# snsinfu/2022a-genome-dynamics

Hardware: AMD Instinct MI355X
Metric: bead-steps/sec on 100kb whole-genome model, 1 GPU and 8-GPU replica farm (higher is better)
Workload: dtype f32

## Files before the change

2022a-genome-dynamics_amd/__init__.py:

```python
from __future__ import annotations

import ctypes as C
import os
from dataclasses import dataclass

import numpy as np

_HERE = os.path.dirname(os.path.abspath(__file__))
LIBGDYN_PATH = os.path.join(_HERE, "csrc", "libgdyn.so")

GD_BOX_OPEN, GD_BOX_PERIODIC = 0, 1
POT_HARMONIC, POT_SPRING, POT_SEMISPRING, POT_SOFTCORE = 0, 1, 2, 3
NOISE_PHILOX, NOISE_ZERO, NOISE_HOST, NOISE_MT19937 = 0, 1, 2, 3
RUN_UPDATE_SCALES, RUN_WALL_DYNAMICS, RUN_DEFER_CALLBACK, RUN_COMPENSATED, RUN_UNCOMPENSATED = 1, 2, 4, 8, 16
ALL_REPLICAS = 0xffffffff
ABI_VERSION = 5
TERM_PAIR, TERM_BOND, TERM_BEND, TERM_POINT, TERM_WALL, TERM_DYNAMIC, TERM_ALL = 1, 2, 4, 8, 16, 32, 63

_STATUS = {1: "GD_EINVAL", 2: "GD_ENODEVICE", 3: "GD_EHIP", 4: "GD_ENOMEM", 5: "GD_ESTATE", 6: "GD_EUNSUPPORTED"}


class GdynError(RuntimeError):
    def __init__(self, code, msg):
        super().__init__(f"{_STATUS.get(code, code)}: {msg}")
# ... 302 lines not shown
        return out

    def forces(self, terms=TERM_ALL):
        out = np.empty((self.R, self.N, 3))
        self.lib.check(self.lib.dll.gd_compute_forces(self._h, terms, _dptr(out)))
        return out

    def search_pairs(self, dcut, replica=0):
        n = C.c_uint64(0)
        self.lib.check(self.lib.dll.gd_search_pairs(self._h, replica, dcut, None, 0, C.byref(n)))
        out = np.empty((n.value, 2), dtype=np.uint32)
        if n.value:
            self.lib.check(self.lib.dll.gd_search_pairs(self._h, replica, dcut, _uptr(out), n.value, C.byref(n)))
        return out

    def contacts_update(self, distance):
        self.lib.check(self.lib.dll.gd_contacts_update(self._h, distance))

    def contacts(self, replica=0):
        n = C.c_uint64(0)
        self.lib.check(self.lib.dll.gd_contacts_fetch(self._h, replica, None, 0, C.byref(n)))
        out = np.empty((n.value, 3), dtype=np.uint32)
        if n.value:
            self.lib.check(self.lib.dll.gd_contacts_fetch(self._h, replica, _uptr(out), n.value, C.byref(n)))
        return out

    def contacts_clear(self, replica=ALL_REPLICAS):
        self.lib.check(self.lib.dll.gd_contacts_clear(self._h, replica))

    def set_tuning(self, skin=0.0, rebuild_interval=0, adapt_interval=1, list_width=0, kernel_path=0, near_fraction=0.0, auto_skin=0):
        t = Tuning(skin, rebuild_interval, adapt_interval, list_width, kernel_path, near_fraction, auto_skin)
        self.lib.check(self.lib.dll.gd_set_tuning(self._h, C.byref(t)))

    def timing(self):
        t = Timing()
        self.lib.check(self.lib.dll.gd_get_timing(self._h, C.byref(t)))
        return t

    def debug_bench(self, what, n=20):
        f = getattr(self.lib.dll, "gd_debug_bench", None)
        if f is None:
            raise GdynError(6, "gd_debug_bench: not in this library (developer builds only: make -C csrc dev; load('libgdyn_dev.so'))")
        f.argtypes = [C.c_void_p, C.c_int, C.c_int, C.POINTER(C.c_double)]
        ms = C.c_double(0)
        self.lib.check(f(self._h, what, n, C.byref(ms)))
        return ms.value

    def stream(self):
        p = C.c_void_p()
        self.lib.check(self.lib.dll.gd_get_stream(self._h, C.byref(p)))
        return p.value
```

2022a-genome-dynamics_amd/csrc/gdyn_capi.hip:

```cpp
#include <algorithm>
#include <cmath>
#include <cstdarg>
#include <cstdio>
#include <cstdlib>
#include <cstring>
#include <new>
#include <string>
#include <vector>

#include "../../include/gdyn.h"
#include "../../include/gdyn_replica.h"
#include "../../include/gdyn_ensemble.h"
#include <hip/hip_fp16.h>

#include "gdyn_types.h"
#include "gdyn_once.hpp"
#include "gdyn_policy.hpp"
#include "gdyn_list.hpp"
#include "gdyn_live.hpp"
#include "gdyn_replica_pairs.hpp"
#include "gdyn_ensemble.hpp"
#include "gdyn_glue.hpp"
#include "gdyn_glue_types.h"
#include "../../include/gdyn_glue.h"
#ifdef GD_DEV
#include "gdyn_dev.h"
#endif


static thread_local char g_err[1024];
static int fail(int code, const char *fmt, ...)
{
    va_list ap;
    va_start(ap, fmt);
    vsnprintf(g_err, sizeof g_err, fmt, ap);
    va_end(ap);
    return code;
}
#define HIPCHK(call)                                                                                    \
    do {                                                                                                \
        hipError_t e_ = (call);                                                                         \
        if (e_ != hipSuccess) return fail(GD_EHIP, "%s failed: %s (%s:%d)", #call, hipGetErrorString(e_), __FILE__, __LINE__); \
    } while (0)
#define GDCHK(call)              \
    do {                         \
// ... 86 lines not shown

    DevBuf<float2> ab_o; uint32_t ab_stride = 0;
    DevBuf<float> mob_o; DevBuf<float4> bendE_o; DevBuf<unsigned char> psmask_o, bdeg_o;
    DevBuf<unsigned> badj_o; DevBuf<int4> chain_o; DevBuf<BondType> btab;
    DevBuf<float4> pos[2], xb, fout, snap;
    DevBuf<unsigned> orig[2], slot_of, rank, members, cell_cnt, cell_start, nbr, meta, badj, flags;
    DevBuf<float> bbox_enc, bbox_w;
    DevBuf<unsigned short> nbr16; DevBuf<TileDesc> tiles;
    DevBuf<float4> rec_x0; DevBuf<uint2> rec_mo; DevBuf<unsigned char> len_prev;
    DevBuf<uint2> wtab, rqueue; DevBuf<unsigned short> need_prev; DevBuf<unsigned> pool;
    DevBuf<float> bbox;
    DevBuf<float2> ab; DevBuf<float> mobs; DevBuf<float4> bendE; DevBuf<int4> chain;
    float mob_uniform = -1.f;
    DevBuf<GridP> grid; DevBuf<DevCtx> ctx[2]; DevBuf<float4> react_part[2]; DevBuf<double> epart;
    DevBuf<unsigned long long> lcount_d; DevBuf<float> noise;
    DevBuf<unsigned long long> seeds_d;
    DevBuf<unsigned> dmax;
    double last_dt = 0, last_kT = -1;
    int last_flags = 0;
    double pend_dt = 0; int pend_flags = 0;
    double near_frac = 0.65;
    DevBuf<uint2> sp_out; DevBuf<unsigned long long> sp_count; std::vector<uint2> sp_host;
    bool sp_valid = false; uint32_t sp_r = 0; double sp_dcut = 0; uint64_t sp_serial = 0;
    DevBuf<unsigned long long> ct_words; DevBuf<unsigned> ct_distinct; size_t ct_cap = 0;
    DevBuf<uint2> ct_pairs; DevBuf<unsigned long long> ct_count; std::vector<unsigned> ct_distinct_h;
    DevBuf<unsigned long long> ct_ck[2]; DevBuf<unsigned> ct_cv[2], ct_n; DevBuf<char> ct_tmp;
    uint64_t state_serial = 1;
    int ocur = 0;
    DevBuf<float4> lo, snap_lo;
    bool lo_valid = false;
    bool comp_last = false;
    double mob_max = 1.0;
    std::vector<hipEvent_t> events;
    ~gd_system()
    {
        for (auto e : events) (void)hipEventDestroy(e);
        if (rp_copied) (void)hipEventDestroy(rp_copied);
        if (stream) (void)hipStreamDestroy(stream);
    }
};

static int valid_pq(int p, int q) { return (p == 2 || p == 4 || p == 6 || p == 8 || p == 12) && q >= 1 && q <= 4; }

extern "C" int gd_abi_version(void) { return GD_ABI_VERSION; }

extern "C" int gd_create_abi(int abi_version, const gd_desc *d, gd_system **out)
{
    if (abi_version != GD_ABI_VERSION)
        return fail(GD_EINVAL, "gd_create: the caller was built against gdyn.h ABI version %d, this library implements %d", abi_version, GD_ABI_VERSION);
    if (!d || !out) return fail(GD_EINVAL, "gd_create: NULL argument");
    if (d->n_beads == 0 || d->n_replicas == 0) return fail(GD_EINVAL, "gd_create: n_beads and n_replicas must be > 0");
    if (d->n_beads > GD_ADJ_MASK) return fail(GD_EINVAL, "gd_create: n_beads exceeds %u", GD_ADJ_MASK);
    if (d->box_kind != GD_BOX_OPEN && d->box_kind != GD_BOX_PERIODIC) return fail(GD_EINVAL, "gd_create: bad box_kind");
    if (d->box_kind == GD_BOX_PERIODIC)
        for (int k = 0; k < 3; k++) if (!(d->box[k] > 0)) return fail(GD_EINVAL, "gd_create: periodic box needs positive periods");
    int ndev = 0;
    if (hipGetDeviceCount(&ndev) != hipSuccess || ndev == 0)
        return fail(GD_ENODEVICE, "gd_create: no HIP device visible (libgdyn has no CPU fallback)");
    if (d->device < 0 || d->device >= ndev) return fail(GD_ENODEVICE, "gd_create: device %d not in [0,%d)", d->device, ndev);
    HIPCHK(hipSetDevice(d->device));
    {
        static gd::DeviceOnce<> once;
        const int rc = once.run(d->device, [](int) { return (int)gd_kernels_init_device(); });
        if (rc != (int)hipSuccess)
            return fail(GD_EHIP, "gd_create: kernel set-up on device %d failed: %s", d->device, rc < 0 ? "device ordinal beyond the guard's table" : hipGetErrorString((hipError_t)rc));
    }
    gd_system *s = new (std::nothrow) gd_system();
    if (!s) return fail(GD_ENOMEM, "gd_create: out of host memory");
    s->N = d->n_beads; s->R = d->n_replicas; s->device = d->device; s->box_kind = d->box_kind;
// ... 457 lines not shown
        if (s->has_scaling) { c.bead_scale = s->bs_init; c.bond_scale = s->bo_init; }
        if (semi) memcpy(c.semi, semi + 3 * r, sizeof c.semi);
    }
    s->ctx_dirty = true; s->list.drop();
    return GD_OK;
}

extern "C" int gd_set_context(gd_system *s, uint32_t r, int64_t step, double bead_scale, double bond_scale, const double semi[3])
{
    if (!s) return fail(GD_EINVAL, "gd_set_context: NULL system");
    if (r >= s->R) return fail(GD_EINVAL, "gd_set_context: replica out of range");
    if (!(bead_scale > 0) || !(bond_scale > 0)) return fail(GD_EINVAL, "gd_set_context: scales must be positive");
    DevCtx &c = s->hctx[r];
    c.step = step; c.bead_scale = bead_scale; c.bond_scale = bond_scale; c.pending = 0;
    if (semi) memcpy(c.semi, semi, sizeof c.semi);
    s->ctx_dirty = true; s->list.drop();
    return GD_OK;
}

extern "C" int gd_set_tuning(gd_system *s, const gd_tuning *t)
{
    if (!s || !t) return fail(GD_EINVAL, "gd_set_tuning: NULL argument");
    if (t->kernel_path > 2) return fail(GD_EINVAL, "gd_set_tuning: kernel_path must be 0..2");
    if (t->near_fraction < 0 || t->near_fraction > 1) return fail(GD_EINVAL, "gd_set_tuning: near_fraction must be in [0,1]");
    HIPCHK(hipSetDevice(s->device));
    if (s->pol.set_tuning(t->skin, t->rebuild_interval, t->adapt_interval, t->list_width, t->auto_skin != 0 || dev_env("GDYN_AUTO_SKIN")))
        (void)s->nbr.resize(0);
    if (t->near_fraction > 0) s->near_frac = t->near_fraction;
    s->kernel_path = t->kernel_path;
    s->list.drop();
    return GD_OK;
}
extern "C" int gd_get_timing(gd_system *s, gd_timing *o) { if (!s || !o) return fail(GD_EINVAL, "gd_get_timing: NULL"); *o = s->timing; return GD_OK; }
extern "C" int gd_get_stream(gd_system *s, void **st) { if (!s || !st) return fail(GD_EINVAL, "gd_get_stream: NULL"); *st = (void *)s->stream; return GD_OK; }


static float pair_cutoff(const gd_system *s)
{
    double m = 0;
    if (s->has_pair) {
        if (s->pair.eps_a != 0 && s->pair.sigma_a > m) m = s->pair.sigma_a;
        if (s->pair.eps_b != 0 && s->pair.sigma_b > m) m = s->pair.sigma_b;
    }
    return (float)m;
}

static int finalize_topology(gd_system *s)
{
    if (!s->topo_dirty) return GD_OK;
    HIPCHK(hipSetDevice(s->device));
    const uint32_t N = s->N;
    std::vector<gd_bond_params> types = s->btypes;
    std::vector<int> terms = s->bterm;
    std::vector<Bond> all = s->bonds;
    for (int d = 0; d < 4; d++) if (s->dyn[d].used) {
        if (types.size() >= GD_MAX_BOND_TYPES) return fail(GD_EINVAL, "too many bond parameter sets");
        types.push_back(s->dyn[d].p); terms.push_back(GD_TERM_DYNAMIC);
        const int t = (int)types.size() - 1;
        for (size_t k = 0; k + 1 < s->dyn[d].pairs.size(); k += 2) all.push_back({s->dyn[d].pairs[k], s->dyn[d].pairs[k + 1], t});
    }
    const bool hetero = !s->ens.homogeneous();
    s->bonds_premixed = false;
    if (!hetero) {
        std::vector<gd_bond_params> t2; std::vector<int> term2; std::vector<Bond> all2 = all;
        bool fits = true, any_mixed = false;
        for (auto &b : all2) {
// ... 80 lines not shown
    s->n_bond_types = (uint32_t)bt.size();
    const size_t RNp = (size_t)s->R * s->Np;
    const uint32_t WBp = std::max((WB + 3u) & ~3u, 4u);
    if (WBp != s->WB || !s->badj.p) { HIPCHK(s->badj.resize((size_t)WBp * RNp)); }
    if (has_bend && !s->chain.p) { HIPCHK(s->chain.resize(RNp)); HIPCHK(s->bendE.resize(RNp)); }
    s->WB = WBp; s->has_bend = has_bend; s->has_bonds = !all.empty();
    s->mob_uniform = (float)s->mob[0];
    for (uint32_t i = 1; i < N; i++) if ((float)s->mob[i] != s->mob_uniform) { s->mob_uniform = -1.f; break; }
    s->mob_max = 0;
    for (uint32_t i = 0; i < N; i++) s->mob_max = std::max(s->mob_max, s->mob[i]);
    s->topo_dirty = false; s->list.topology_changed();
    return GD_OK;
}


static double scale_at(const gd_system *s, double init, double tau, double time) { (void)s; return 1.0 - (1.0 - init) * std::exp(-time / tau); }

static double cut_scale(const gd_system *s, const gd_run_desc *run, uint32_t ahead)
{
    if (!s->pair.scale_by_bead_scale) return 1.0;
    double m = 0;
    for (auto &c : s->hctx) {
        m = std::max(m, c.bead_scale);
        if (run && (run->flags & GD_RUN_UPDATE_SCALES) && s->has_scaling)
            m = std::max(m, scale_at(s, s->bs_init, s->bs_tau, (double)(c.step + ahead + 1) * run->timestep));
    }
    return m;
}

static void fill_common(gd_system *s, StepParams &p)
{
    memset(&p, 0, sizeof p);
    p.N = s->N; p.Np = s->Np; p.R = s->R; p.nblk = s->nblk; p.stride = (size_t)s->R * s->Np;
    set_box(s, p);
    p.pos_in = s->pos[s->pcur].p; p.pos_out = s->pos[s->pcur ^ 1].p; p.xb = s->xb.p; p.orig = s->orig[s->ocur].p;
    p.ab = s->ab.p; p.mob = s->mobs.p; p.bendE = s->bendE.p; p.mob_uniform = s->mob_uniform; p.WB = s->WB;
    p.nbr = s->nbr.p; p.nbr16 = s->nbr16.p; p.wtab = s->wtab.p; p.tiles = s->tiles.p; p.tiled = s->list.tiled ? 1 : 0; p.packed_ab = s->packed_ab ? 1 : 0;
    p.cpb = s->cpb; p.tile_cap = s->list.tiled ? s->list.tile_cap : s->pol.tile_cap;
    p.pk = (s->has_pair && s->pair.p_a == 2 && s->pair.q_a == 3 && s->pair.p_b == 8 && s->pair.q_b == 3) ? (s->pair.mix ? 1 : 2) : 0;
    p.meta = s->meta.p; p.rec_x0 = s->rec_x0.p; p.rec_mo = s->rec_mo.p; p.W = s->list.W; p.badj = s->badj.p; p.chain = s->chain.p;
    p.ctx_in = s->ctx[s->ccur].p; p.ctx_out = s->ctx[s->ccur ^ 1].p; p.flags = s->flags.p;
    p.react_in = s->react_part[s->ccur].p; p.react_out = s->react_part[s->ccur ^ 1].p;
    if (s->has_pair) {
        const gd_pair_softcore &q = s->pair;
        p.pair = PairP{(float)q.eps_a, (float)q.sigma_a, (float)q.eps_b, (float)q.sigma_b, q.p_a, q.q_a, q.p_b, q.q_b,
                       q.mix, q.scale_by_bead_scale, pair_cutoff(s) > 0 ? 1 : 0, pair_cutoff(s)};
    }
    if (s->has_wall) {
        const gd_wall &w = s->wall;
        p.wall.eps_a = (float)w.eps_a; p.wall.sigma_a = (float)w.sigma_a; p.wall.eps_b = (float)w.eps_b; p.wall.sigma_b = (float)w.sigma_b;
        p.wall.p_a = w.p_a; p.wall.q_a = w.q_a; p.wall.p_b = w.p_b; p.wall.q_b = w.q_b;
        p.wall.wall_a = (float)w.wall_a_factor; p.wall.wall_b = (float)w.wall_b_factor; p.wall.scaled = w.scale_by_bead_scale;
        p.wall.enabled = 1; p.wall.packing_spring = (float)w.packing_spring;
        p.wall.fast2383 = (w.p_a == 2 && w.q_a == 3 && w.p_b == 8 && w.q_b == 3) ? 1 : 0;
        for (int k = 0; k < 3; k++) p.wall.spring[k] = w.semiaxes_spring[k];
        p.wall.mobility = w.mobility;
    }
    if (s->has_inner) {
        const gd_inner_sphere &w = s->inner;
        p.wall.inner_enabled = 1; p.wall.in_radius = (float)w.radius;
        p.wall.in_eps_a = (float)w.eps_a; p.wall.in_sigma_a = (float)w.sigma_a; p.wall.in_eps_b = (float)w.eps_b; p.wall.in_sigma_b = (float)w.sigma_b;
        p.wall.in_p_a = w.p_a; p.wall.in_q_a = w.q_a; p.wall.in_p_b = w.p_b; p.wall.in_q_b = w.q_b;
        p.wall.in_wall_a = (float)w.wall_a_factor; p.wall.in_wall_b = (float)w.wall_b_factor; p.wall.in_spring = (float)w.spring;
    }
    p.scaling = ScaleP{s->has_scaling ? 1 : 0, 0, s->bs_init, s->bs_tau, s->bo_init, s->bo_tau, 0.0, 0.0};
    p.btab = s->btab.p; p.nbt = (int)s->n_bond_types; p.has_softcore_bonds = s->has_softcore_bonds ? 1 : 0;
// ... 177 lines not shown
    fill_common(s, p);
    p.dt_d = s->pend_dt; p.dt = (float)s->pend_dt; p.run_flags = s->pend_flags;
    bool common = s->has_scaling && (s->pend_flags & GD_RUN_UPDATE_SCALES);
    for (uint32_t r = 1; r < s->R && common; r++) common = s->hctx[r].step == s->hctx[0].step && s->hctx[r].pending == s->hctx[0].pending;
    if (common) {
        const double time = (double)(s->hctx[0].step + 1) * s->pend_dt;
        p.scaling.from_host = 1;
        p.scaling.bead_next = scale_at(s, s->bs_init, s->bs_tau, time);
        p.scaling.bond_next = scale_at(s, s->bo_init, s->bo_tau, time);
    }
    gd_launch_finalize(p, 0, s->stream);
    s->ccur ^= 1;
    GDCHK(download_ctx(s));
    s->state_serial++;
    return GD_OK;
}

static bool want_compensated(const gd_system *s, const gd_run_desc *run)
{
    if (run->flags & GD_RUN_UNCOMPENSATED) return false;
    if (run->flags & GD_RUN_COMPENSATED) return true;
    double X = 0;
    if (s->has_wall) for (auto &c : s->hctx) for (int k = 0; k < 3; k++) X = std::max(X, c.semi[k]);
    if (s->box_kind == GD_BOX_PERIODIC) for (int k = 0; k < 3; k++) X = std::max(X, s->box[k]);
    if (!(X > 0)) X = 16.0;
    const double ulp = std::ldexp(1.0, std::ilogb(X) - 23), sigma = std::sqrt(2.0 * s->mob_max * run->temperature * run->timestep);
    return sigma < 64.0 * ulp;
}

extern "C" int gd_apply_callback(gd_system *s)
{
    if (!s) return fail(GD_EINVAL, "gd_apply_callback: NULL system");
    return apply_pending(s);
}

static int enqueue_chunk(gd_system *s, const gd_run_desc *run, int64_t done, bool comp, bool host_noise, Chunk &c)
{
    const size_t RN = (size_t)s->R * s->N;
    const bool with_list = pair_cutoff(s) > 0;
    const int64_t chunk = c.steps = s->pol.chunk_steps(run->steps - done);
    gd_launch_gather_positions(s->pos[s->pcur].p, s->slot_of.p, s->snap.p, s->N, s->Np, s->R, 0, s->stream);
    if (comp) HIPCHK(hipMemcpyAsync(s->snap_lo.p, s->lo.p, RN * sizeof(float4), hipMemcpyDeviceToDevice, s->stream));
    c.snap_ctx = s->hctx; c.snap_w_packed = s->list.w_packed;
    GDCHK(clear_flags(s));
    StepParams p;
    bool common_step = s->has_scaling && (run->flags & GD_RUN_UPDATE_SCALES);
    const long long step0 = s->hctx[0].step;
    for (uint32_t r = 1; r < s->R && common_step; r++) common_step = s->hctx[r].step == step0;
    auto host_scales = [&](StepParams &q, int64_t launch) {
        if (!common_step) return;
        const double time = (double)(step0 + launch) * run->timestep;
        q.scaling.from_host = 1;
        q.scaling.bead_next = scale_at(s, s->bs_init, s->bs_tau, time);
        q.scaling.bond_next = scale_at(s, s->bo_init, s->bo_tau, time);
    };
    size_t nev = 0;
    HIPCHK(hipEventRecord(get_event(s, nev++), s->stream));
    int64_t k = 0;
    c.on_search_list = s->list.valid && s->list.search_list;
    while (k < chunk) {
        if (!s->list.valid || s->list.steps_since_build >= s->pol.K) {
            s->pol.take_pending_skin(pair_cutoff(s));
            hipEvent_t e1 = get_event(s, nev++);
            GDCHK(enqueue_build(s, list_radius(s, run, (uint32_t)(k + s->pol.K)), with_list));
            s->list.enter_use(false);
            HIPCHK(hipEventRecord(e1, s->stream));
            c.spans.push_back({nev - 1, 1});
        }
        const int64_t n = std::min<int64_t>((int64_t)s->pol.K - s->list.steps_since_build, chunk - k);
        hipEvent_t e1 = get_event(s, nev++);
        for (int64_t q = 0; q < n; q++) {
            fill_common(s, p);
            p.dt_d = run->timestep; p.dt = (float)run->timestep; p.kT = (float)run->temperature; p.seed = run->seed;
            p.seeds = run->replica_seeds ? s->seeds_d.p : nullptr;
            p.noise_mode = run->noise_mode; p.run_flags = run->flags; p.comp = comp ? 1 : 0;
            p.host_noise = host_noise ? s->noise.p + (size_t)(done + k + q) * RN * 3 : nullptr;
            host_scales(p, k + q);
            p.record_disp = (s->list.steps_since_build + (uint32_t)q + 1u == s->pol.K);
            c.full_interval |= p.record_disp != 0;
            gd_launch_step(p, GD_MODE_STEP, s->stream);
            if (s->sw_n) launch_softwell(s, p, 0);
            if (s->rp.any()) launch_replica_pairs(s, p, 0);
            s->pcur ^= 1; s->ccur ^= 1;
        }
        HIPCHK(hipEventRecord(e1, s->stream));
        c.spans.push_back({nev - 1, 0});
        s->timing.step_launches += (uint64_t)n;
        s->list.stepped((uint32_t)n);
        k += n;
    }
    const bool defer = (run->flags & GD_RUN_DEFER_CALLBACK) && done + chunk == run->steps;
    if (!defer) {
        fill_common(s, p);
        p.dt_d = run->timestep; p.dt = (float)run->timestep; p.run_flags = run->flags;
        host_scales(p, chunk);
        gd_launch_finalize(p, 0, s->stream);
        s->ccur ^= 1;
    } else {
        s->pend_dt = run->timestep; s->pend_flags = run->flags;
        if (s->has_wall) {
            fill_common(s, p);
            p.ctx_out = s->ctx[s->ccur].p;
            gd_launch_finalize(p, 1, s->stream);
        }
    }
    c.ev_end = nev;
    HIPCHK(hipEventRecord(get_event(s, nev++), s->stream));
    return GD_OK;
}

static int rollback_chunk(gd_system *s, const Chunk &c, bool over, bool comp, int retries)
{
    const size_t RN = (size_t)s->R * s->N;
    s->rollbacks++;
    HIPCHK(hipMemcpy2DAsync(s->pos[s->pcur].p, (size_t)s->Np * sizeof(float4), s->snap.p, (size_t)s->N * sizeof(float4),
                            (size_t)s->N * sizeof(float4), s->R, hipMemcpyDeviceToDevice, s->stream));
    gd_launch_identity(s->orig[s->ocur].p, s->slot_of.p, s->N, s->Np, s->R, s->stream);
// ... 24 lines not shown
        HIPCHK(hipEventElapsedTime(&ms, s->events[sp.first - 1], s->events[sp.first]));
        (sp.second ? build_ms : step_ms) += ms;
    }
    HIPCHK(hipEventElapsedTime(&ms, s->events[0], s->events[c.ev_end]));
    s->timing.total_ms += ms; s->timing.step_kernel_ms += step_ms; s->timing.rebuild_ms += build_ms;
    s->hctx = c.ctx;
    unsigned long long L = 0; for (uint32_t r = 0; r < s->R; r++) L += s->lcount[r];
    s->timing.list_entries_visited += L * (uint64_t)c.steps;
    const gd::Accepted a{ms, c.steps, c.rep.maxd2, cut_scale(s, nullptr, 0), c.full_interval, c.on_search_list};
    if (s->pol.on_accepted(list_state(s), a, [&](uint32_t ahead) { return cut_scale(s, run, ahead); })) s->list.drop();
    return GD_OK;
}

extern "C" int gd_run(gd_system *s, const gd_run_desc *run)
{
    if (!s || !run) return fail(GD_EINVAL, "gd_run: NULL argument");
    if (run->spacestep != 0) return fail(GD_EUNSUPPORTED, "gd_run: spacestep != 0 (adaptive timestep) is not supported");
    if (run->steps < 0 || !(run->timestep > 0) || run->temperature < 0) return fail(GD_EINVAL, "gd_run: bad steps/timestep/temperature");
    if (run->noise_mode < 0 || run->noise_mode > GD_NOISE_HOST)
        return fail(run->noise_mode == 3 ? GD_EUNSUPPORTED : GD_EINVAL, "gd_run: noise_mode %d not available on the device", run->noise_mode);
    if (run->noise_mode == GD_NOISE_HOST && !run->host_noise) return fail(GD_EINVAL, "gd_run: host noise requested without array");
    if ((run->flags & GD_RUN_WALL_DYNAMICS) && !s->has_wall) return fail(GD_ESTATE, "gd_run: wall dynamics requested without a wall");
    if ((run->flags & GD_RUN_UPDATE_SCALES) && !s->has_scaling) return fail(GD_ESTATE, "gd_run: scale updates requested without gd_set_scaling");
    GDCHK(prepare(s));
    GDCHK(apply_pending(s));
    s->state_serial++;
    if (run->timestep != s->last_dt || run->temperature != s->last_kT) { s->pol.a2_ema = 0; s->last_dt = run->timestep; s->last_kT = run->temperature; }
    if (s->pol.adapt && s->pol.K > 4 && ((run->flags ^ s->last_flags) & (GD_RUN_WALL_DYNAMICS | GD_RUN_UPDATE_SCALES)) != 0 && s->rebuilds > 0)
        s->pol.K -= s->pol.K / 5;
    s->last_flags = run->flags;
    const bool with_list = pair_cutoff(s) > 0;
    const size_t RN = (size_t)s->R * s->N;
    memset(&s->timing, 0, sizeof s->timing);

    const bool host_noise = run->noise_mode == GD_NOISE_HOST && run->temperature > 0;
    if (host_noise) {
        const size_t n = (size_t)run->steps * RN * 3;
        std::vector<float> h(n);
        for (size_t i = 0; i < n; i++) h[i] = (float)run->host_noise[i];
        HIPCHK(s->noise.resize(n, false));
        HIPCHK(hipMemcpy(s->noise.p, h.data(), n * sizeof(float), hipMemcpyHostToDevice));
    }

    const bool comp = run->steps > 0 && want_compensated(s, run);
    if (comp) {
        if (!s->lo_valid) { HIPCHK(hipMemsetAsync(s->lo.p, 0, RN * sizeof(float4), s->stream)); s->lo_valid = true; }
        HIPCHK(s->snap_lo.resize(RN, false));
    }
    if (run->steps > 0) s->comp_last = comp;
    if (run->steps > 0 && !comp) s->lo_valid = false;

    if (run->replica_seeds) {
        static_assert(sizeof(unsigned long long) == sizeof(uint64_t), "seed width");
        HIPCHK(s->seeds_d.resize(s->R, false));
        HIPCHK(hipMemcpy(s->seeds_d.p, run->replica_seeds, s->R * sizeof(uint64_t), hipMemcpyHostToDevice));
    }

    int64_t done = 0;
    int retries = 0;
    s->pol.retries_over(false);
    float last_dmax2 = 0;
    while (done < run->steps) {
        Chunk c;
        GDCHK(enqueue_chunk(s, run, done, comp, host_noise, c));
        GDCHK(read_chunk(s, c));
        const bool over = s->pol.on_report(list_state(s), c.rep);
// ... 496 lines not shown
```

2022a-genome-dynamics_amd/csrc/gdyn_kernels.hip:

```cpp
#include <hip/hip_fp16.h>

#include <algorithm>

#include "gdyn_types.h"

#include "gdyn_stamps.h"

#if GD_ABL == 40 || GD_ABL == 41 || GD_ABL == 43
#define GD_REPLAY 1
constexpr bool RP_MEM = (GD_ABL == 40), RP_ALU = (GD_ABL == 41 || GD_ABL == 43);
#define GD_CONSUME4(v) asm volatile("" :: "v"((v).x), "v"((v).y), "v"((v).z), "v"((v).w))
#define GD_LAUNDER4(v) asm volatile("" : "+v"((v).x), "+v"((v).y), "+v"((v).z), "+v"((v).w))
#endif

#define TERM_PAIR 1u
#define TERM_BOND 2u
#define TERM_BEND 4u
#define TERM_POINT 8u
#define TERM_WALL 16u
#define TERM_DYNAMIC 32u
#define RUN_UPDATE_SCALES 1
#define RUN_WALL_DYNAMICS 2
#define NOISE_PHILOX 0
#define NOISE_ZERO 1
// ... 408 lines not shown
    const float mu_dt = mu * p.dt;
    const float sg = s_ctx.sg_uniform >= 0.f ? s_ctx.sg_uniform : sqrtf(2.0f * p.kT * mu_dt);
    const float ex = mu_dt * F.x + sg * z.x, ey = mu_dt * F.y + sg * z.y, ez = mu_dt * F.z + sg * z.z;
    float nx = xi.x + ex, ny = xi.y + ey, nz = xi.z + ez;
    if (p.comp) {
        float4 *lp = p.lo + ((size_t)r * p.N + bead.oid);
        const float4 l = *lp;
        const float tx = l.x + ex, ty = l.y + ey, tz = l.z + ez;
        nx = xi.x + tx; ny = xi.y + ty; nz = xi.z + tz;
        const float bx = nx - xi.x, by = ny - xi.y, bz = nz - xi.z;
        *lp = make_float4((xi.x - (nx - bx)) + (tx - bx), (xi.y - (ny - by)) + (ty - by), (xi.z - (nz - bz)) + (tz - bz), 0.f);
    }
    if (TILED) *(float4 *)((char *)(p.pos_out + bead.rbase + (size_t)blk * GD_BLOCK) + bead.local * 16u) = make_float4(nx, ny, nz, bead.xi4.w);
    else p.pos_out[bead.g] = make_float4(nx, ny, nz, bead.xi4.w);
    float dnew2 = 0.f;
    if (TILED) { const float e2 = ex * ex + ey * ey + ez * ez; dnew2 = (disp2 + e2 + 2.0f * __builtin_amdgcn_sqrtf(disp2 * e2)) * 1.000002f; }
    return dnew2;
}

template <int MODE, bool PERIODIC, bool TILED, int PK, bool S16, bool SPLIT = false>
#ifndef GD_STEP_WAVES
#define GD_STEP_WAVES 8
#endif
__global__ __launch_bounds__(GD_BLOCK, (TILED && MODE == GD_MODE_STEP) ? (S16 ? GD_STEP_WAVES : 4) : 1) void k_step(const StepParams p)
{
    extern __shared__ __attribute__((aligned(16))) float4 s_tile[];
    __shared__ BondType s_bt[GD_MAX_BOND_TYPES];
    __shared__ CtxF s_ctx;
    __shared__ float s_red[GD_BLOCK / 64][4];
    __shared__ double s_e[GD_BLOCK / 64];

    unsigned r, blk;
    if (!block_map(blockIdx.x, p.nblk, p.cpb, r, blk)) return;
    if (TILED && SPLIT) {
        const unsigned held = p.tiles[(size_t)r * p.nblk + blk].total;
        if (held <= p.tile_lo || held > p.tile_hi) return;
    }
    const unsigned tid = threadIdx.x, lane = tid & 63, wid = tid >> 6;
    const size_t rbase = (size_t)r * p.Np;
    const float4 *__restrict__ rpos = p.pos_in + rbase;

    GD_STAMP_BEGIN();
    const long long ctx_step0 = p.ctx_in[r].step;
    const int ctx_pending0 = p.ctx_in[r].pending;
    const float dmax0 = (MODE == GD_MODE_STEP && TILED) ? __uint_as_float(p.dmax[r * GD_DMAX_STRIDE]) : 0.f;
    const size_t gw6 = (rbase + blk * GD_BLOCK) / 64 + (size_t)(unsigned)__builtin_amdgcn_readfirstlane((int)wid);
    const uint2 wrow = TILED ? p.wtab[gw6] : make_uint2(0u, 0u);
    const unsigned NCL = TILED ? wrow.y : p.W / 4, NCB = p.WB / 4;
    uint2 mo = make_uint2(0u, 0u);
    float4 rec = make_float4(0.f, 0.f, 0.f, 0.f);
    uint4 adj0 = make_uint4(0, 0, 0, 0), qa = adj0, qb = adj0;
    unsigned own_base = 0, tile_ok = 0;
    if (TILED) {
        const size_t tbase = rbase + (size_t)blk * GD_BLOCK;
        mo = *(const uint2 *)((const char *)(p.rec_mo + tbase) + tid * 8u);
        const TileDesc *td = p.tiles + (size_t)r * p.nblk + blk;
        unsigned tlen[GD_TILE_RANGES], tst[GD_TILE_RANGES];
#pragma unroll
        for (int k = 0; k < GD_TILE_RANGES; k++) { tlen[k] = td->len[k]; tst[k] = td->start[k]; }
        own_base = td->own_base; tile_ok = td->nranges;
        asm volatile("" : "+v"(mo.x), "+v"(mo.y));
        GD_STAMP(9);
        {
            constexpr bool W0_FREE = MODE == GD_MODE_STEP;
            const unsigned wq = (unsigned)__builtin_amdgcn_readfirstlane((int)((W0_FREE ? (wid == 0 ? 0x100000u : wid - 1u) : wid) * 64u));
            constexpr unsigned DMA_STRIDE = W0_FREE ? GD_BLOCK - 64u : GD_BLOCK;
// ... 400 lines not shown
            const float4 v = p.react_in[(size_t)r * p.nblk + b];
            rx += v.x; ry += v.y; rz += v.z;
        }
        c.react[0] = wave_sum_d(rx); c.react[1] = wave_sum_d(ry); c.react[2] = wave_sum_d(rz);
    } else if (c.pending) {
        apply_callback(c, p, r, lane);
    }
    if (lane == 0) p.ctx_out[r] = c;
}

typedef void (*StepKernel)(StepParams);
template <int MODE, bool SPLIT, bool PER, bool TIL, bool S16>
static StepKernel step_kernel_pk(int pk)
{
    return pk == 1 ? k_step<MODE, PER, TIL, 1, S16, SPLIT> : pk == 2 ? k_step<MODE, PER, TIL, 2, S16, SPLIT> : k_step<MODE, PER, TIL, 0, S16, SPLIT>;
}
template <int MODE, bool SPLIT>
static StepKernel tiled_step_kernel(bool periodic, int pk, bool s16)
{
    static_assert(!SPLIT || MODE == GD_MODE_STEP, "only stepping is split by tile class");
    if (periodic) return s16 ? step_kernel_pk<MODE, SPLIT, true, true, true>(pk) : step_kernel_pk<MODE, SPLIT, true, true, false>(pk);
    return s16 ? step_kernel_pk<MODE, SPLIT, false, true, true>(pk) : step_kernel_pk<MODE, SPLIT, false, true, false>(pk);
}
template <int MODE>
static StepKernel step_kernel(bool periodic, bool tiled, int pk, bool s16)
{
    if (tiled) return tiled_step_kernel<MODE, false>(periodic, pk, s16);
    return periodic ? step_kernel_pk<MODE, false, true, false, false>(pk) : step_kernel_pk<MODE, false, false, false, false>(pk);
}

template <int MODE>
static void launch_step_mode(const StepParams &p, hipStream_t st)
{
    const dim3 grid(p.cpb ? GD_XCDS * p.cpb * p.R : p.R * p.nblk), block(GD_BLOCK);
    const size_t lds = p.tiled ? (size_t)p.tile_cap * sizeof(float4) : 0;
    const bool s16 = p.tiled && gd_tile_s16(p.tile_cap);
    const unsigned split_at = !p.tiled ? 0u : (s16 && p.tile_cap > 3312u) ? 3312u : (!s16 && p.tile_cap > 5072u) ? 5072u : (!s16 && p.tile_cap > 3312u) ? 3312u : 0u;
    if (MODE == GD_MODE_STEP && split_at) {
        const StepKernel k = tiled_step_kernel<GD_MODE_STEP, true>(p.periodic, p.pk, s16);
        StepParams q = p;
        for (int half = 0; half < 2; half++) {
            q.tile_cap = half ? p.tile_cap : split_at; q.tile_lo = half ? split_at : 0u; q.tile_hi = half ? 0xffffffffu : split_at;
            hipLaunchKernelGGL(k, grid, block, (size_t)q.tile_cap * sizeof(float4), st, q);
        }
        return;
    }
    const StepKernel k = step_kernel<MODE>(p.periodic, p.tiled, p.pk, s16);
    hipLaunchKernelGGL(k, grid, block, lds, st, p);
}

void gd_launch_step(const StepParams &p, int mode, hipStream_t st)
{
    if (mode == GD_MODE_STEP) launch_step_mode<GD_MODE_STEP>(p, st);
    else if (mode == GD_MODE_FORCE) launch_step_mode<GD_MODE_FORCE>(p, st);
    else launch_step_mode<GD_MODE_ENERGY>(p, st);
}

void gd_launch_finalize(const StepParams &p, int mode, hipStream_t st)
{
    hipLaunchKernelGGL(k_ctx, dim3(p.R), dim3(64), 0, st, p, mode);
}


template <int CTRL, int ROW_MASK>
__device__ __forceinline__ float dppi(float v, float ident)
{
    return __int_as_float(__builtin_amdgcn_update_dpp(__float_as_int(ident), __float_as_int(v), CTRL, ROW_MASK, 0xf, false));
// ... 1357 lines not shown
```

2022a-genome-dynamics_amd/csrc/gdyn_policy.hpp:

```cpp
#pragma once
#include <algorithm>
#include <cmath>
#include <cstdint>
#include <cstdio>
#include <cstring>
#include <vector>

#include "gdyn_types.h"

namespace gd {

struct BuildReport {
    unsigned bits = 0;
    bool over = false, class_over = false, tile_over = false, violated = false;
    unsigned need_w = 0, need_t = 0, ncell = 0;
    float maxd2 = 0;
};

inline BuildReport summarize(const unsigned *flags, uint32_t R)
{
    BuildReport b;
    for (const unsigned *f = flags; f < flags + (size_t)R * GD_NFLAGS; f += GD_NFLAGS) {
        b.bits |= f[GD_FLAG_OVERFLOW]; b.tile_over |= f[GD_FLAG_TILE_OVERFLOW] != 0; b.violated |= f[GD_FLAG_VIOLATION] != 0;
        b.need_w = std::max(b.need_w, f[GD_FLAG_NEED_W]); b.need_t = std::max(b.need_t, f[GD_FLAG_NEED_TILE]); b.ncell = std::max(b.ncell, f[GD_FLAG_NCELL]);
        float d2; memcpy(&d2, &f[GD_FLAG_MAXDISP2], 4); b.maxd2 = std::max(b.maxd2, d2);
    }
    b.over = b.bits != 0; b.class_over = (b.bits & 2u) != 0;
    return b;
}

struct ListState {
    double cut = 0;
    float rv = 0;
    bool tiled = false;
    uint32_t tile_cap = 0, W = 0;
    uint32_t pool_used = 0; size_t pool_kib = 0;
    double rows = 0;
    bool droplet = false, can_tile = false;
};

struct Accepted { double ms = 0; int64_t steps = 0; float maxd2 = 0; double scale_now = 1; bool full_interval = false, on_search_list = false; };

struct PoolPlan {
    size_t used = 0;
    size_t want = 0;
    bool resize = false;
    size_t alloc_kib = 0;
};
inline PoolPlan plan_pool(size_t pool_used, size_t pool_kib, size_t waves, uint32_t W, bool predict)
{
    PoolPlan pl;
    pl.used = std::max<size_t>(pool_used, predict ? waves : waves * std::max<size_t>(W / 8u, 1u));
    pl.want = pl.used + pl.used / 8 + 2 * waves;
    pl.resize = pool_kib < pl.want || pool_kib > 2 * pl.want + 4 * waves;
    pl.alloc_kib = pl.want + pl.want / 16;
    return pl;
}

struct ListPolicy {
    std::vector<unsigned> tile_caps = {3312u, 4080u, 5072u, 8192u};
    double k_target = 0.90;
    FILE *trace = nullptr;
    size_t mem_total = 0;
    double skin = 0.75;
    bool skin_fixed = false;
    double skin_next = 0;
    double skin_dense_from = 0;
    bool dense_by_tile = false;
    uint32_t dense_budget = 0;
    uint32_t skin_streak = 0, skin_hold = 0;
    uint32_t K = 4, adapt = 1, K_bad = 0, K_bad_ttl = 0;
    double a2_ema = 0;
    uint32_t W = 0, tile_cap = 3312, tile_hold = 0;
    bool all_near = false;
    bool tiled_ok = true; uint32_t tiled_off = 0;
    uint32_t tiled_wait = 0, tiled_backoff = 8;
    uint32_t repair_wide = 0;
    uint32_t last_need_w = 0, last_need_t = 0;
    uint32_t ncell_seen = 0;
    struct SkinTuner {
        bool enabled = false, done = false;
        std::vector<double> cand, cost; size_t idx = 0;
        int settle = 0, measured = 0, wait = 4, rounds = 0;
        uint32_t K_ref = 0, cap_ref = 0;
        double acc_ms = 0; uint64_t acc_steps = 0;
    } tuner;

    bool want_tiled(bool can_tile) const { return can_tile && tiled_ok && W <= GD_TILED_MAX_W; }
    int64_t chunk_steps(int64_t left) const
// ... 244 lines not shown
```

2022a-genome-dynamics_amd/csrc/gdyn_types.h:

```cpp
#pragma once
#include <hip/hip_runtime.h>
#include <stdint.h>

#ifndef GD_BLOCK
#define GD_BLOCK 512
#endif
#define GD_MAX_BOND_TYPES 16
#define GD_MAX_POINT_SOURCES 4
#define GD_ADJ_SHIFT 26
#define GD_ADJ_MASK ((1u << GD_ADJ_SHIFT) - 1u)
#define GD_ADJ_LOCAL 0x80000000u
#define GD_CHAIN_LOCAL 0x40000000
#define GD_TILE_RANGES 9
#define GD_XCDS 8
#define GD_REC_NOBEAD 0xffffffffu
#define GD_TILED_MAX_NEAR 8184u
#define GD_TILED_MAX_FAR 504u
#define GD_TILED_MAX_W (GD_TILED_MAX_NEAR + GD_TILED_MAX_FAR)
inline bool gd_tile_s16(unsigned tile_cap) { return tile_cap < 4096u; }
#define GD_REC_ID_MASK 0x03ffffffu
#define GD_DMAX_STRIDE 32u
#define GD_REPAIR_GRID 1024u
#define GD_UNROLL 8u

// ... 61 lines not shown
    int fast2383;
    float packing_spring;
    double spring[3], mobility;
    int inner_enabled;
    float in_radius, in_eps_a, in_sigma_a, in_eps_b, in_sigma_b, in_wall_a, in_wall_b, in_spring;
    int in_p_a, in_q_a, in_p_b, in_q_b;
};

struct BondType {
    float ka, kb, la, lb;
    int flags;
    float xmin;
    int kind;
    int pq;
};

struct PointSrc {
    int kind;
    float k, b, p[3];
};

struct ScaleP {
    int enabled;
    int from_host;
    double bead_init, bead_tau, bond_init, bond_tau;
    double bead_next, bond_next;
};

struct StepParams {
    unsigned N, Np, R, nblk;
    size_t stride;
    int periodic;
    float box[3], inv_box[3];
    const float4 *pos_in;
    float4 *pos_out;
    const float4 *xb;
    const unsigned *orig;
    const float2 *ab;
    const float *mob;
    const float4 *bendE;
    const unsigned *nbr;
    const unsigned short *nbr16;
    const TileDesc *tiles;
    const uint2 *wtab;
    const unsigned *meta;
    unsigned W, WB;
    float mob_uniform;
    int tiled;
    int pk;
    int packed_ab;
    unsigned cpb;
    unsigned tile_cap;
    unsigned tile_lo, tile_hi;
    const float4 *rec_x0;
    const uint2 *rec_mo;
    int has_softcore_bonds;
    int bonds_premixed;
    int bonds_all_scaled;
    const unsigned *badj;
    const int4 *chain;
    const DevCtx *ctx_in;
    DevCtx *ctx_out;
    const float4 *react_in;
    float4 *react_out;
    unsigned *flags;
    PairP pair;
    WallP wall;
    ScaleP scaling;
    const BondType *btab;
    int nbt;
    PointSrc ps[GD_MAX_POINT_SOURCES];
    int nps;
    int has_bend, has_bonds;
    double dt_d;
    float dt, kT;
    unsigned long long seed;
    const unsigned long long *seeds;
    int noise_mode, run_flags;
    const float *host_noise;
    float rv;
    float rn;
    unsigned *dmax;
    int record_disp;
    float4 *lo;
    int comp;
    unsigned term_mask;
    float4 *fout;
    double *epart;
};

struct BuildParams {
    unsigned N, Np, R, nblk;
    size_t stride;
    int periodic;
    float box[3], inv_box[3];
    float rv;
    float rn;
    unsigned *dmax;
    unsigned ncell_cap;
    unsigned scan_segments;
    int kx;
    const float4 *pos_in;
    float4 *pos_out;
    float4 *xb;
    const unsigned *orig_in;
    unsigned *orig_out;
    unsigned *slot_of;
    unsigned *rank;
    unsigned *members;
    unsigned *cell_cnt, *cell_start;
    float *bbox;
    const float *bbox_cur;
    float *bbox_next;
    float *bbox_w;
    int warm;
    GridP *grid;
// ... 112 lines not shown
```

Measured before the change: 25.07 billion.

## Split step launches into two replica groups on concurrent streams

When the neighbour list is tiled, noise is generated on the device, the replica map is whole-replica and the pair potential uses the fast path, the per-step launch is split by replica range into two groups. One group runs on the main stream and the other on a second non-blocking stream, with fork and join events around each chunk. Because replicas are independent, each group can proceed through its steps without waiting for the other, which is meant to reduce launch tails and idle compute units between dependent launches. The cost is extra event and stream bookkeeping, and each launch has fewer blocks. The grid size is now taken from a replica count, and an offset is added to the replica index in the tiled packed kernel path.

```diff
diff --git a/2022a-genome-dynamics_amd/__init__.py b/2022a-genome-dynamics_amd/__init__.py
--- a/2022a-genome-dynamics_amd/__init__.py
+++ b/2022a-genome-dynamics_amd/__init__.py
@@ -358,6 +358,24 @@
         t = Tuning(skin, rebuild_interval, adapt_interval, list_width, kernel_path, near_fraction, auto_skin)
         self.lib.check(self.lib.dll.gd_set_tuning(self._h, C.byref(t)))
 
+    def _groups_fn(self, name):
+        f = getattr(self.lib.dll, name, None)
+        if f is None:
+            raise GdynError(6, f"{name}: not in this library (include/gdyn_groups.h: csrc/libgdyn.so only)")
+        return f
+
+    def set_step_groups(self, mode=0):
+        f = self._groups_fn("gd_set_step_groups")
+        f.argtypes = [C.c_void_p, C.c_uint32]
+        self.lib.check(f(self._h, mode))
+
+    def step_groups(self):
+        f = self._groups_fn("gd_get_step_groups")
+        f.argtypes = [C.c_void_p, C.POINTER(C.c_uint32), C.POINTER(C.c_uint32)]
+        mode, last = C.c_uint32(0), C.c_uint32(0)
+        self.lib.check(f(self._h, C.byref(mode), C.byref(last)))
+        return mode.value, last.value
+
     def timing(self):
         t = Timing()
         self.lib.check(self.lib.dll.gd_get_timing(self._h, C.byref(t)))
diff --git a/2022a-genome-dynamics_amd/csrc/gdyn_capi.hip b/2022a-genome-dynamics_amd/csrc/gdyn_capi.hip
--- a/2022a-genome-dynamics_amd/csrc/gdyn_capi.hip
+++ b/2022a-genome-dynamics_amd/csrc/gdyn_capi.hip
@@ -11,6 +11,7 @@
 #include "../../include/gdyn.h"
 #include "../../include/gdyn_replica.h"
 #include "../../include/gdyn_ensemble.h"
+#include "../../include/gdyn_groups.h"
 #include <hip/hip_fp16.h>
 
 #include "gdyn_types.h"
@@ -163,9 +164,14 @@
     bool comp_last = false;
     double mob_max = 1.0;
     std::vector<hipEvent_t> events;
+    hipStream_t stream2 = nullptr; hipEvent_t grp_fork = nullptr, grp_join = nullptr;
+    uint32_t group_mode = gd::STEP_GROUPS_RULE, groups_last = 1;
     ~gd_system()
     {
         for (auto e : events) (void)hipEventDestroy(e);
+        if (grp_fork) (void)hipEventDestroy(grp_fork);
+        if (grp_join) (void)hipEventDestroy(grp_join);
+        if (stream2) (void)hipStreamDestroy(stream2);
         if (rp_copied) (void)hipEventDestroy(rp_copied);
         if (stream) (void)hipStreamDestroy(stream);
     }
@@ -689,6 +695,21 @@
     return GD_OK;
 }
 extern "C" int gd_get_timing(gd_system *s, gd_timing *o) { if (!s || !o) return fail(GD_EINVAL, "gd_get_timing: NULL"); *o = s->timing; return GD_OK; }
+extern "C" int gd_groups_abi_version(void) { return GD_GROUPS_ABI_VERSION; }
+extern "C" int gd_set_step_groups(gd_system *s, uint32_t mode)
+{
+    if (!s) return fail(GD_EINVAL, "gd_set_step_groups: NULL system");
+    if (mode > gd::STEP_GROUPS_TWO) return fail(GD_EINVAL, "gd_set_step_groups: mode must be 0 (rule), 1 (one launch) or 2 (two groups wherever results allow)");
+    s->group_mode = mode;
+    return GD_OK;
+}
+extern "C" int gd_get_step_groups(gd_system *s, uint32_t *mode, uint32_t *last_groups)
+{
+    if (!s) return fail(GD_EINVAL, "gd_get_step_groups: NULL system");
+    if (mode) *mode = s->group_mode;
+    if (last_groups) *last_groups = s->groups_last;
+    return GD_OK;
+}
 extern "C" int gd_get_stream(gd_system *s, void **st) { if (!s || !st) return fail(GD_EINVAL, "gd_get_stream: NULL"); *st = (void *)s->stream; return GD_OK; }
 
 
@@ -835,6 +856,7 @@
 {
     memset(&p, 0, sizeof p);
     p.N = s->N; p.Np = s->Np; p.R = s->R; p.nblk = s->nblk; p.stride = (size_t)s->R * s->Np;
+    p.r0 = 0; p.nrep = s->R;
     set_box(s, p);
     p.pos_in = s->pos[s->pcur].p; p.pos_out = s->pos[s->pcur ^ 1].p; p.xb = s->xb.p; p.orig = s->orig[s->ocur].p;
     p.ab = s->ab.p; p.mob = s->mobs.p; p.bendE = s->bendE.p; p.mob_uniform = s->mob_uniform; p.WB = s->WB;
@@ -1078,6 +1100,35 @@
 {
     if (!s) return fail(GD_EINVAL, "gd_apply_callback: NULL system");
     return apply_pending(s);
+}
+
+static int fork_groups(gd_system *s)
+{
+    if (!s->stream2) HIPCHK(hipStreamCreateWithFlags(&s->stream2, hipStreamNonBlocking));
+    if (!s->grp_fork) HIPCHK(hipEventCreateWithFlags(&s->grp_fork, hipEventDisableTiming));
+    if (!s->grp_join) HIPCHK(hipEventCreateWithFlags(&s->grp_join, hipEventDisableTiming));
+    HIPCHK(hipEventRecord(s->grp_fork, s->stream));
+    HIPCHK(hipStreamWaitEvent(s->stream2, s->grp_fork, 0));
+    return GD_OK;
+}
+static int join_groups(gd_system *s)
+{
+    hipError_t e = hipEventRecord(s->grp_join, s->stream2);
+    if (e == hipSuccess) e = hipStreamWaitEvent(s->stream, s->grp_join, 0);
+    if (e != hipSuccess) {
+        (void)hipStreamSynchronize(s->stream2);
+        return fail(GD_EHIP, "gd_run: joining the step groups failed: %s", hipGetErrorString(e));
+    }
+    return GD_OK;
+}
+
+static gd::StepGroupState group_state(const gd_system *s, bool host_noise)
+{
+    gd::StepGroupState st;
+    st.R = s->R; st.nblk = s->nblk; st.tiled = s->list.valid && s->list.tiled; st.post_step = post_step_active(s);
+    st.device_noise = !host_noise; st.whole_replica_map = s->cpb == 0;
+    st.fast_pair = s->has_pair && s->pair.p_a == 2 && s->pair.q_a == 3 && s->pair.p_b == 8 && s->pair.q_b == 3;
+    return st;
 }
 
 static int enqueue_chunk(gd_system *s, const gd_run_desc *run, int64_t done, bool comp, bool host_noise, Chunk &c)
@@ -1115,6 +1166,11 @@
         }
         const int64_t n = std::min<int64_t>((int64_t)s->pol.K - s->list.steps_since_build, chunk - k);
         hipEvent_t e1 = get_event(s, nev++);
+        uint32_t min_blocks = gd::STEP_GROUPS_MIN_BLOCKS, a16 = gd::STEP_GROUPS_A16;
+        if (const char *e = dev_env("GDYN_GROUP_MIN_BLOCKS")) min_blocks = (uint32_t)atoi(e);
+        if (const char *e = dev_env("GDYN_GROUP_A16")) a16 = (uint32_t)atoi(e);
+        const uint32_t ra = gd::step_group_split(s->group_mode, group_state(s, host_noise), min_blocks, a16);
+        if (ra) { GDCHK(fork_groups(s)); s->groups_last = 2; }
         for (int64_t q = 0; q < n; q++) {
             fill_common(s, p);
             p.dt_d = run->timestep; p.dt = (float)run->timestep; p.kT = (float)run->temperature; p.seed = run->seed;
@@ -1124,11 +1180,15 @@
             host_scales(p, k + q);
             p.record_disp = (s->list.steps_since_build + (uint32_t)q + 1u == s->pol.K);
             c.full_interval |= p.record_disp != 0;
-            gd_launch_step(p, GD_MODE_STEP, s->stream);
+            if (ra) {
+                p.r0 = 0; p.nrep = ra; gd_launch_step(p, GD_MODE_STEP, s->stream);
+                p.r0 = ra; p.nrep = s->R - ra; gd_launch_step(p, GD_MODE_STEP, s->stream2);
+            } else gd_launch_step(p, GD_MODE_STEP, s->stream);
             if (s->sw_n) launch_softwell(s, p, 0);
             if (s->rp.any()) launch_replica_pairs(s, p, 0);
             s->pcur ^= 1; s->ccur ^= 1;
         }
+        if (ra) GDCHK(join_groups(s));
         HIPCHK(hipEventRecord(e1, s->stream));
         c.spans.push_back({nev - 1, 0});
         s->timing.step_launches += (uint64_t)n;
@@ -1219,6 +1279,7 @@
     const bool with_list = pair_cutoff(s) > 0;
     const size_t RN = (size_t)s->R * s->N;
     memset(&s->timing, 0, sizeof s->timing);
+    s->groups_last = 1;
 
     const bool host_noise = run->noise_mode == GD_NOISE_HOST && run->temperature > 0;
     if (host_noise) {
diff --git a/2022a-genome-dynamics_amd/csrc/gdyn_kernels.hip b/2022a-genome-dynamics_amd/csrc/gdyn_kernels.hip
--- a/2022a-genome-dynamics_amd/csrc/gdyn_kernels.hip
+++ b/2022a-genome-dynamics_amd/csrc/gdyn_kernels.hip
@@ -464,6 +464,7 @@
 
     unsigned r, blk;
     if (!block_map(blockIdx.x, p.nblk, p.cpb, r, blk)) return;
+    if (MODE == GD_MODE_STEP && TILED && PK != 0) r += p.r0;
     if (TILED && SPLIT) {
         const unsigned held = p.tiles[(size_t)r * p.nblk + blk].total;
         if (held <= p.tile_lo || held > p.tile_hi) return;
@@ -930,7 +931,7 @@
 template <int MODE>
 static void launch_step_mode(const StepParams &p, hipStream_t st)
 {
-    const dim3 grid(p.cpb ? GD_XCDS * p.cpb * p.R : p.R * p.nblk), block(GD_BLOCK);
+    const dim3 grid(p.cpb ? GD_XCDS * p.cpb * p.nrep : p.nrep * p.nblk), block(GD_BLOCK);
     const size_t lds = p.tiled ? (size_t)p.tile_cap * sizeof(float4) : 0;
     const bool s16 = p.tiled && gd_tile_s16(p.tile_cap);
     const unsigned split_at = !p.tiled ? 0u : (s16 && p.tile_cap > 3312u) ? 3312u : (!s16 && p.tile_cap > 5072u) ? 5072u : (!s16 && p.tile_cap > 3312u) ? 3312u : 0u;
diff --git a/2022a-genome-dynamics_amd/csrc/gdyn_policy.hpp b/2022a-genome-dynamics_amd/csrc/gdyn_policy.hpp
--- a/2022a-genome-dynamics_amd/csrc/gdyn_policy.hpp
+++ b/2022a-genome-dynamics_amd/csrc/gdyn_policy.hpp
@@ -55,6 +55,30 @@
     pl.resize = pool_kib < pl.want || pool_kib > 2 * pl.want + 4 * waves;
     pl.alloc_kib = pl.want + pl.want / 16;
     return pl;
+}
+
+enum : uint32_t { STEP_GROUPS_RULE = 0, STEP_GROUPS_ONE = 1, STEP_GROUPS_TWO = 2 };
+struct StepGroupState {
+    uint32_t R = 0, nblk = 0;
+    bool tiled = false;
+    bool post_step = false;
+    bool device_noise = true;
+    bool whole_replica_map = false;
+    bool fast_pair = false;
+};
+constexpr uint32_t STEP_GROUPS_MIN_BLOCKS = 384u;
+constexpr uint32_t STEP_GROUPS_A16 = 8u;
+inline uint32_t step_group_split(uint32_t mode, const StepGroupState &st, uint32_t min_blocks = STEP_GROUPS_MIN_BLOCKS, uint32_t a16 = STEP_GROUPS_A16)
+{
+    if (mode != STEP_GROUPS_RULE && mode != STEP_GROUPS_TWO) return 0;
+    if (!st.tiled || st.post_step || !st.device_noise || !st.whole_replica_map || !st.fast_pair) return 0;
+    if (st.R < 2 * GD_XCDS || st.R % GD_XCDS != 0 || st.nblk == 0) return 0;
+    a16 = std::min(std::max(a16, 1u), 15u);
+    uint32_t ra = (uint32_t)(((uint64_t)st.R * a16 + 8u * GD_XCDS) / (16u * GD_XCDS)) * GD_XCDS;
+    ra = std::min(std::max(ra, (uint32_t)GD_XCDS), st.R - GD_XCDS);
+    const uint32_t small = std::min(ra, st.R - ra);
+    if (mode == STEP_GROUPS_RULE && (uint64_t)small * st.nblk < min_blocks) return 0;
+    return ra;
 }
 
 struct ListPolicy {
diff --git a/2022a-genome-dynamics_amd/csrc/gdyn_types.h b/2022a-genome-dynamics_amd/csrc/gdyn_types.h
--- a/2022a-genome-dynamics_amd/csrc/gdyn_types.h
+++ b/2022a-genome-dynamics_amd/csrc/gdyn_types.h
@@ -117,6 +117,7 @@
     size_t stride;
     int periodic;
     float box[3], inv_box[3];
+    unsigned r0;
     const float4 *pos_in;
     float4 *pos_out;
     const float4 *xb;
@@ -167,6 +168,7 @@
     float rn;
     unsigned *dmax;
     int record_disp;
+    unsigned nrep;
     float4 *lo;
     int comp;
     unsigned term_mask;
diff --git a/include/gdyn_groups.h b/include/gdyn_groups.h
--- /dev/null
+++ b/include/gdyn_groups.h
@@ -0,0 +1,22 @@
+#ifndef GDYN_GROUPS_H
+#define GDYN_GROUPS_H
+
+#include <stdint.h>
+
+#include "gdyn.h"
+
+#ifdef __cplusplus
+extern "C" {
+#endif
+
+#define GD_GROUPS_ABI_VERSION 1
+
+int gd_groups_abi_version(void);
+int gd_set_step_groups(gd_system *sys, uint32_t mode);
+int gd_get_step_groups(gd_system *sys, uint32_t *mode, uint32_t *last_groups);
+
+#ifdef __cplusplus
+}
+#endif
+
+#endif
```

Result: faster. 25.69 billion, median of 6 (+2.5%).
